# MerlinPCarson/WakeWord-Detection

Measured on AMD Instinct MI355X. Metric: audio frames/sec (16 kHz, 40-mel, 10 ms hop) + FRR@0.5 FA/h, higher is better.
Workload: dtype f32; 1 GPU; CRNN forward, batch=256x1.5 s synthetic 16 kHz clips per GPU, PCM resident in HBM -> log-mel (fp64 FFT) -> 151x40 window -> encode+detect, fp32 MFMA; clips_per_gpu=256, samples_per_clip=24000, resident_input_batches_rotated=24, resident_input_bytes=294912000, pipelined_contexts=4, weights=reference tf_lite_models (shipped fp32 weights), parallelism=single GPU

## Files before the change

wakeword-detection_amd/csrc/crnn.hip:

```cpp
#include "stream_fe.h"
#include <algorithm>
#include <type_traits>

#include <cstdlib>

typedef float f32x4 __attribute__((ext_vector_type(4)));

struct win_addr {
  const int64_t *row;
  const int32_t *valid;
  int64_t row0;
  int hop;
  int valid_const;
  int64_t mel_rows;
};

__device__ __forceinline__ void window_span(const win_addr &wa, int w, int T, int64_t &row, int &valid) {
  if (wa.row && wa.valid) {
    const int64_t r = wa.row[w];
    const int v = wa.valid[w];
    row = r;
    valid = v;
  } else {
    row = wa.row ? wa.row[w] : wa.row0 + (int64_t)w * wa.hop;
// ... 274 lines not shown
    load_a(av[0], 0);                                                                                \
    _Pragma("unroll") for (int i = 0; i < NT_; ++i) {                                                \
      if (i + 1 < NT_) load_a(av[(i + 1) & 1], i + 1);                                               \
      __builtin_amdgcn_sched_barrier(0);                                                             \
      f32x4 acc0 = {cb0, cb0, cb0, cb0}, acc1 = {cb1, cb1, cb1, cb1};                                \
      CV_MFMA_KB(av[i & 1], 0) CV_MFMA_KB(av[i & 1], 1) CV_MFMA_KB(av[i & 1], 2)                     \
      __builtin_amdgcn_sched_barrier(0);                                                             \
      __VA_ARGS__                                                                                    \
      __builtin_amdgcn_sched_barrier(0);                                                             \
      CV_MFMA_KB(av[i & 1], 3) CV_MFMA_KB(av[i & 1], 4) CV_MFMA_KB(av[i & 1], 5) CV_MFMA_LAST(av[i & 1]) \
      prev0 = acc0;                                                                                  \
      prev1 = acc1;                                                                                  \
    }                                                                                                \
  }

#define PJ_KS_BYTES (4 * 192 * 16)
typedef const __attribute__((address_space(1))) char *pj_gptr;
typedef const __attribute__((address_space(1))) f32x4 *pj_gptr4;
__device__ __forceinline__ float4 pj_w_ld(pj_gptr4 p) {
  const f32x4 v = *p;
  return make_float4(v.x, v.y, v.z, v.w);
}
#define PJ_W_LANE(wx1s_)                                                                             \
  const pj_gptr wb_0 = (pj_gptr)(wx1s_);                                                             \
  unsigned wb_lane = (unsigned)((kk * 192 + wave * 48 + j) * 16);
#define PJ_W_KSTEP(wk_, ks_)                                                                         \
  pj_gptr wk_ = wb_0 + (size_t)(ks_) * PJ_KS_BYTES;                                                  \
  asm("" : "+s"(wk_));                                                                               \
  asm("" : "+v"(wb_lane));
#define PJ_W_LD(wk_, n_) pj_w_ld((pj_gptr4)(wk_ + wb_lane + (n_) * 256))
#define PJ_RING_PROLOGUE(DEPTH_)                                                                     \
  _Pragma("unroll") for (int s2 = 0; s2 < DEPTH_ - 1; ++s2) {                                        \
    PJ_W_KSTEP(wk, s2)                                                                               \
    _Pragma("unroll") for (int n = 0; n < 3; ++n) bq[s2][n] = PJ_W_LD(wk, n);                        \
  }
#define PJ_LOAD_BIAS(bv1_, bx1_)                                                                     \
  _Pragma("unroll") for (int n = 0; n < 3; ++n) bv1_[n] = (bx1_)[wave * 48 + n * 16 + j];
#define PJ_ROWS16(e_)                                                                                \
  acc[0] = __builtin_amdgcn_mfma_f32_16x16x4f32(avq[ks & 1].e_, b[0].e_, acc[0], 0, 0, 0);            \
  acc[1] = __builtin_amdgcn_mfma_f32_16x16x4f32(avq[ks & 1].e_, b[1].e_, acc[1], 0, 0, 0);            \
  acc[2] = __builtin_amdgcn_mfma_f32_16x16x4f32(avq[ks & 1].e_, b[2].e_, acc[2], 0, 0, 0);
#define PJ_ROWS3(e_)                                                                                 \
  rem[0] = __builtin_amdgcn_mfma_f32_4x4x1f32(rvq[ks & 1].e_, b[0].e_, rem[0], 0, 0, 0);              \
  rem[1] = __builtin_amdgcn_mfma_f32_4x4x1f32(rvq[ks & 1].e_, b[1].e_, rem[1], 0, 0, 0);              \
  rem[2] = __builtin_amdgcn_mfma_f32_4x4x1f32(rvq[ks & 1].e_, b[2].e_, rem[2], 0, 0, 0);
#define PJ_NO_ROWS(e_)
#define PJ_KLOOP(DEPTH_, G16_, G3_, ...)                                                             \
  _Pragma("unroll") for (int ks = 0; ks < 40; ++ks) {                                                \
    if (ks + DEPTH_ - 1 < 40) {                                                                      \
      PJ_W_KSTEP(wk, ks + DEPTH_ - 1)                                                                \
      _Pragma("unroll") for (int n = 0; n < 3; ++n) bq[(ks + DEPTH_ - 1) % DEPTH_][n] = PJ_W_LD(wk, n); \
    }                                                                                                \
    if (ks + 1 < 40) { __VA_ARGS__ }                                                                 \
    __builtin_amdgcn_sched_barrier(0);                                                               \
    const float4 *b = bq[ks % DEPTH_];                                                               \
    G16_(x) G3_(x) G16_(y) G3_(y) G16_(z) G3_(z) G16_(w) G3_(w)                                      \
    __builtin_amdgcn_sched_barrier(0);                                                               \
  }
#define PJ_REM_ROWS(rem_, bv_, ...)                                                                  \
  _Pragma("unroll") for (int i = 0; i < 3; ++i) {                                                    \
    float s3 = rem_[i];                                                                              \
    s3 += __shfl_xor(s3, 16);                                                                        \
    s3 += __shfl_xor(s3, 32);                                                                        \
    if (kk == 0) {                                                                                   \
      const float v = s3 + bv_;                                                                      \
      __VA_ARGS__                                                                                    \
    }                                                                                                \
  }

#define CF_THREADS 256
#define CF_FLD 648
#define CF_IMG_FLOATS (CV_ROWS * CV_LDT)
#define CF_FEAT_FLOATS (CV_OT * CF_FLD)
#define CF_SMEM_BYTES ((CF_IMG_FLOATS + CF_FEAT_FLOATS) * 4)
#define CF_NO_ROW (-0x40000000)
#define CF_FUSED_FEAT_ROWS 13
#define CF_FUSED_SMEM_BYTES ((CF_IMG_FLOATS + CF_FUSED_FEAT_ROWS * CF_FLD) * 4)
#define CF_ALIAS_ROWS0 24
#define CF_ALIAS_REM (CF_ALIAS_ROWS0 + 3 * CF_FLD)
static_assert((((CF_ALIAS_ROWS0 - CF_IMG_FLOATS) / 4 - 2 * 13) % 16 + 16) % 16 == 0 && CF_IMG_FLOATS % 4 == 0, "aliased rows off their bank slots");
static_assert(CV_OT - 16 == 3 && 16 - CF_FUSED_FEAT_ROWS == 3 && CF_ALIAS_REM + 20 * 96 <= 20 * GR_GX_LD ,
              "the aliased rows must lie under gx");
#define CF_GX 0
#define CF_SEQ (20 * GR_GX_LD)
#define CF_HB (CF_SEQ + 32 * GR_SEQ_LD)
#define CF_ENC (CF_HB + 2 * 2 * 2 * GR_H)
#define CF_HID (CF_ENC + 2 * GR_H)
#define CF_W2S (CF_HID + 2 * GR_H)
static_assert(CF_W2S + 8 * 64 <= CF_IMG_FLOATS, "post-conv LDS layout exceeds the image region");
static_assert(64 * GR_W1_LD <= CF_FEAT_FLOATS && 16 * 192 * 4 <= CF_FEAT_FLOATS, "feat region too small for its later tenants");
static_assert(64 * GR_W1_LD <= CF_FUSED_FEAT_ROWS * CF_FLD, "fused kernel's feat region too small for the head's first layer");

struct fused_args {
  const float *mel;
  win_addr wa;
  const float *w4;
  const float *cbias;
  const float *wx1s;
  const float *bx1;
  const float *wh1, *bh1;
  const float *wx2s;
  const float *bx2, *wh2, *bh2, *w1, *b1, *w2, *b2;
  float *enc;
  float *out;
  int T, NOUT, HEAD;
  long long *stamps;
  float *gx_out;
  const unsigned short *cwb;
  const unsigned short *wx1b;
  ww_tick_tag tag;
};

template <bool SEQ>
__device__ __forceinline__ float cf_recurrence(const gru_w &g, const float *gxs, float *hd, float *seq1, int dir, int unit, int half) {
  constexpr int H = GR_H, OT = CV_OT;
  static_assert(OT % 2 == 1, "the step loop is pairs of steps plus one");
  const int t0 = dir ? OT - 1 : 0;
  const int gx_step = dir ? -GR_GX_LD : GR_GX_LD, seq_step = dir ? -GR_SEQ_LD : GR_SEQ_LD;
  const float *gxp = gxs + t0 * GR_GX_LD + dir * 3 * H + unit;
  float *sqp = SEQ ? seq1 + t0 * GR_SEQ_LD + dir * H + unit : nullptr;
  float *hw = hd + unit;
  float h_own = 0.f;
  float gz = gxp[0], gr = gxp[H], gc = gxp[2 * H];
#pragma unroll 1
  for (int s = 0; s < OT / 2; ++s) {
    float nz, nr, nc;
    gxp += gx_step;
    h_own = gru_step<true>(g, hd, half, gz, gr, gc, h_own, gxp, nz, nr, nc);
    if (half == 0) {
      hw[H] = h_own;
      if (SEQ) *sqp = h_own;
    }
    if (SEQ) sqp += seq_step;
    wsync_h();
    gxp += gx_step;
    h_own = gru_step<true>(g, hd + H, half, nz, nr, nc, h_own, gxp, gz, gr, gc);
    if (half == 0) {
      hw[0] = h_own;
      if (SEQ) *sqp = h_own;
    }
    if (SEQ) sqp += seq_step;
    wsync_h();
  }
  float nz, nr, nc;
  h_own = gru_step<false>(g, hd, half, gz, gr, gc, h_own, nullptr, nz, nr, nc);
  if (half == 0) {
    hw[H] = h_own;
    if (SEQ) *sqp = h_own;
  }
  wsync_h();
  return h_own;
}

#define CF_ROUND_L2(av_, rv_, b_, e_)                                                                  \
  acc[0] = __builtin_amdgcn_mfma_f32_16x16x4f32(av_.e_, b_[0].e_, acc[0], 0, 0, 0);                     \
  acc[1] = __builtin_amdgcn_mfma_f32_16x16x4f32(av_.e_, b_[1].e_, acc[1], 0, 0, 0);                     \
  acc[2] = __builtin_amdgcn_mfma_f32_16x16x4f32(av_.e_, b_[2].e_, acc[2], 0, 0, 0);                     \
  rem[0] = __builtin_amdgcn_mfma_f32_16x16x4f32(rv_.e_, b_[0].e_, rem[0], 0, 0, 0);                     \
  rem[1] = __builtin_amdgcn_mfma_f32_16x16x4f32(rv_.e_, b_[1].e_, rem[1], 0, 0, 0);                     \
  rem[2] = __builtin_amdgcn_mfma_f32_16x16x4f32(rv_.e_, b_[2].e_, rem[2], 0, 0, 0);

#define L2_LOAD_W(bq_, wx2s_, nt0_)                                                                  \
  _Pragma("unroll") for (int kb = 0; kb < 4; ++kb)                                                   \
    _Pragma("unroll") for (int n = 0; n < 3; ++n)                                                    \
      bq_[kb][n] = *(const float4 *)((wx2s_) + ((size_t)(kb * 4 + kk) * 192 + ((nt0_) + n) * 16 + j) * 4);
#define L2_LOAD_BIAS(bb_, bx2_, nt0_) \
  _Pragma("unroll") for (int n = 0; n < 3; ++n) bb_[n] = (bx2_)[((nt0_) + n) * 16 + j];
#define L2_PROJECT(bq_, bb_, rrow_, nt0_, ...)                                                       \
  {                                                                                                  \
    f32x4 acc[3] = {{0.f, 0.f, 0.f, 0.f}, {0.f, 0.f, 0.f, 0.f}, {0.f, 0.f, 0.f, 0.f}};               \
    f32x4 rem[3] = {{0.f, 0.f, 0.f, 0.f}, {0.f, 0.f, 0.f, 0.f}, {0.f, 0.f, 0.f, 0.f}};               \
    _Pragma("unroll") for (int kb = 0; kb < 4; ++kb) {                                               \
      const float4 av = *(const float4 *)(&seq1[j * GR_SEQ_LD + kb * 16 + kk * 4]);                  \
      const float4 rv = *(const float4 *)(&seq1[(rrow_) * GR_SEQ_LD + kb * 16 + kk * 4]);            \
      const float4 *b = bq_[kb];                                                                     \
      CF_ROUND_L2(av, rv, b, x) CF_ROUND_L2(av, rv, b, y) CF_ROUND_L2(av, rv, b, z) CF_ROUND_L2(av, rv, b, w) \
    }                                                                                                \
    __VA_ARGS__                                                                                      \
    _Pragma("unroll") for (int n = 0; n < 3; ++n) {                                                  \
      const int col = ((nt0_) + n) * 16 + j;                                                         \
      const float bb = bb_[n];                                                                       \
      _Pragma("unroll") for (int r = 0; r < 4; ++r) gxs[(kk * 4 + r) * GR_GX_LD + col] = acc[n][r] + bb; \
      if (kk == 0) {                                                                                 \
        _Pragma("unroll") for (int r = 0; r < 3; ++r) gxs[(16 + r) * GR_GX_LD + col] = rem[n][r] + bb; \
      }                                                                                              \
    }                                                                                                \
  }

__device__ __forceinline__ void cf_phases_d_to_g(const fused_args &a, float *img, float *feat, const gru_w &g, int w) {
  constexpr int H = GR_H;
  const int tid = threadIdx.x, lane = tid & 63, wave = wave_index(tid);
  const int j = lane & 15, kk = lane >> 4;
  const int unit = lane >> 1, half = lane & 1, dir = wave & 1;
  float *gxs = img + CF_GX, *seq1 = img + CF_SEQ, *hb = img + CF_HB, *encs = img + CF_ENC, *hid = img + CF_HID, *w2s = img + CF_W2S;
  float4 bq2[4][3];
  L2_LOAD_W(bq2, a.wx2s, wave * 3)
  if (wave < 2) {
    __builtin_amdgcn_s_setprio(3);
    cf_recurrence<true>(g, gxs, hb + dir * 2 * H, seq1, dir, unit, half);
    __builtin_amdgcn_s_setprio(0);
  }
  __syncthreads();

  {
    float bb2[3];
    L2_LOAD_BIAS(bb2, a.bx2, wave * 3)
    __builtin_amdgcn_sched_barrier(0);
    L2_PROJECT(bq2, bb2, 16 + j, wave * 3, )
  }
  __syncthreads();

  float *w1s = feat;
  if (wave >= 2) {
    __builtin_amdgcn_s_setprio(3);
    const float h_last = cf_recurrence<false>(g, gxs, hb + (2 + dir) * 2 * H, nullptr, dir, unit, half);
    __builtin_amdgcn_s_setprio(0);
    if (half == 0) {
      encs[dir * H + unit] = h_last;
      if (a.enc) a.enc[(size_t)w * 2 * H + dir * H + unit] = h_last;
    }
  } else {
    for (int i = tid; i < 64 * 64; i += 128) w1s[(i >> 6) * GR_W1_LD + (i & 63)] = a.w1[i];
    for (int i = tid; i < a.NOUT * 64; i += 128) w2s[i] = a.w2[i];
  }
  __syncthreads();

  if (wave == 0) {
    const float b1v = a.b1[lane], b2v = a.b2[lane < a.NOUT ? lane : 0];
    __builtin_amdgcn_sched_barrier(0);
    float acc = 0.f;
#pragma unroll 16
    for (int k = 0; k < 2 * H; ++k) acc = fmaf(w1s[lane * GR_W1_LD + k], encs[k], acc);
    hid[lane] = fmaxf(acc + b1v, 0.f);
    wsync_g();
    float y = 0.f;
    if (lane < a.NOUT) {
      for (int k = 0; k < 2 * H; ++k) y = fmaf(w2s[lane * 64 + k], hid[k], y);
      y += b2v;
    }
    const float p = head_activation(y, lane, a.NOUT, a.HEAD);
    if (a.tag.slots) {
      if (lane == a.tag.pidx) tick_tag_store(a.tag, w, p);
    } else if (lane < a.NOUT) {
      a.out[(size_t)w * a.NOUT + lane] = p;
    }
  }
}

#define CF_STAMP(i_) \
  if (FRONT_ONLY && a.stamps && lane == 0) a.stamps[((size_t)blockIdx.x * 4 + wave) * 10 + (i_)] = __builtin_amdgcn_s_memtime();
__device__ __forceinline__ void cf_set_move(fused_args &a, long long off) {
  ww_set_move(a.w4, off); ww_set_move(a.cbias, off); ww_set_move(a.wx1s, off); ww_set_move(a.bx1, off);
  ww_set_move(a.wh1, off); ww_set_move(a.bh1, off); ww_set_move(a.wx2s, off); ww_set_move(a.bx2, off);
  ww_set_move(a.wh2, off); ww_set_move(a.bh2, off); ww_set_move(a.w1, off); ww_set_move(a.b1, off);
  ww_set_move(a.w2, off); ww_set_move(a.b2, off); ww_set_move(a.cwb, off); ww_set_move(a.wx1b, off);
}
template <bool FRONT_ONLY, bool SET = false>
__global__ __launch_bounds__(CF_THREADS, 2) void crnn_fused_kernel(fused_args a, ww_set_ref set) {
  if constexpr (SET) cf_set_move(a, ww_set_offset(set, blockIdx.x));
  extern __shared__ __align__(16) float cf_smem[];
  float *img = cf_smem, *feat = cf_smem + CF_IMG_FLOATS;
  constexpr int H = GR_H, OT = CV_OT;
  const int tid = threadIdx.x, lane = tid & 63, wave = tid >> 6;
  const int j = lane & 15, kk = lane >> 4;
  const int w = blockIdx.x;
  CF_STAMP(0)
  int64_t row;
  int valid;
  window_span(a.wa, w, a.T, row, valid);

  float4 wreg[CV_KB][2];
  float wlast[2], cb0, cb1;
  CV_LOAD_W(wreg, wlast, cb0, cb1, a.w4, a.cbias)

  int a_off[6], o_off[6][4];
  {
    constexpr int MAXV = 6;
    const float *src = a.mel + row * CV_NMEL;
    const int n = valid * CV_NMEL;
    const bool al16 = ((((uintptr_t)src) & 15) == 0);
    float4 stage[MAXV];
    if (n > 0)
      stage_loads(al16, [&](auto al) {
        constexpr bool AL = decltype(al)::value;
#pragma unroll
        for (int q = 0; q < MAXV; ++q) {
          const int i = (q * CF_THREADS + tid) * 4;
          stage[q] = ld_mel4<AL>(src + (i < n ? i : n - 4), true);
        }
      });
    LDS_CLEAR16(img, CF_IMG_FLOATS / 4, CF_THREADS)
#pragma unroll
    for (int i = 0; i < 6; ++i) {
      constexpr int M = CV_OT * CV_OF;
      const int mt = wave + 4 * i;
      int m = mt * 16 + j;
      if (m >= M) m = M - 1;
      const int t = m / CV_OF, f = m - t * CV_OF;
      a_off[i] = (f * CV_SF) * CV_LDT + t * CV_ST;
#pragma unroll
      for (int r = 0; r < 4; ++r) {
        const int mo = mt * 16 + kk * 4 + r;
        const int to = mo / CV_OF, fo = mo - to * CV_OF;
        if (i < 4) o_off[i][r] = to * CF_FLD + fo * 32 + j;
        else if (i == 4) o_off[i][r] = (to < 13 ? to * CF_FLD : CF_ALIAS_ROWS0 - CF_IMG_FLOATS + (to - 13) * CF_FLD) + fo * 32 + j;
        else o_off[i][r] = mo >= M ? CF_NO_ROW : CF_ALIAS_REM - CF_IMG_FLOATS + fo * 96 + 16 * (to - 16) + j;
      }
    }
    __syncthreads();
#pragma unroll
    for (int q = 0; q < MAXV; ++q) {
      const int i = (q * CF_THREADS + tid) * 4;
      if (i < n) {
        const int it = i / CV_NMEL, im = i - it * CV_NMEL;
        float *d = img + (im + CV_PF) * CV_LDT + it + CV_PT;
        d[0] = stage[q].x;
        d[CV_LDT] = stage[q].y;
        d[2 * CV_LDT] = stage[q].z;
        d[3 * CV_LDT] = stage[q].w;
      }
    }
  }
  __syncthreads();
  CF_STAMP(1)
  PJ_W_LANE(a.wx1s)
  float4 bq[4][3];
  {
    auto load_a = [&](cv_a &av, int i) { CV_LOAD_A(av, img + a_off[i]) };
    auto store_tile = [&](int i, const f32x4 &r0, const f32x4 &r1) {
#pragma unroll
      for (int r = 0; r < 4; ++r) {
        if (i < 5) {
          feat[o_off[i][r]] = relu1(r0[r]);
          feat[o_off[i][r] + 16] = relu1(r1[r]);
        } else if (o_off[i][r] != CF_NO_ROW) {
          feat[o_off[i][r]] = relu1(r0[r]);
          feat[o_off[i][r] + 48] = relu1(r1[r]);
        }
      }
    };
    f32x4 prev0 = {0.f, 0.f, 0.f, 0.f}, prev1 = {0.f, 0.f, 0.f, 0.f}, t4_0 = prev0, t4_1 = prev0;
    CV_TILE_LOOP(6, if (i > 0 && i < 5) store_tile(i - 1, prev0, prev1); if (i == 5) { t4_0 = prev0; t4_1 = prev1; })
    PJ_RING_PROLOGUE(4)
    __builtin_amdgcn_sched_barrier(0);
    lds_barrier();
    store_tile(4, t4_0, t4_1);
    store_tile(5, prev0, prev1);
  }
  CF_STAMP(2)
  lds_barrier();
  CF_STAMP(3)
  float *gxs = img + CF_GX, *seq1 = img + CF_SEQ, *hb = img + CF_HB;
  CLEAR_SEQ_H(seq1, 32, hb, CF_THREADS)

  const int unit = lane >> 1, half = lane & 1, dir = wave & 1;
  gru_w g;
  {
    const float *a0p = (j < 13 ? feat + j * CF_FLD : img + CF_ALIAS_ROWS0 + (j - 13) * CF_FLD) + kk * 4;
    const int r1 = (lane & 3) < 3 ? (lane & 3) : 2;
    const float *a1p = img + CF_ALIAS_REM + 16 * r1 + kk * 4;
    f32x4 acc[3] = {{0.f, 0.f, 0.f, 0.f}, {0.f, 0.f, 0.f, 0.f}, {0.f, 0.f, 0.f, 0.f}};
// ... 502 lines not shown
          const bf16x8_t wh = __builtin_bit_cast(bf16x8_t, wq[0][ks][mt]), wl = __builtin_bit_cast(bf16x8_t, wq[1][ks][mt]);
          acc[mt] = __builtin_amdgcn_mfma_f32_16x16x32_bf16(wl, xh[i & 1][ks], acc[mt], 0, 0, 0);
          acc[mt] = __builtin_amdgcn_mfma_f32_16x16x32_bf16(wh, xl[i & 1][ks], acc[mt], 0, 0, 0);
          acc[mt] = __builtin_amdgcn_mfma_f32_16x16x32_bf16(wh, xh[i & 1][ks], acc[mt], 0, 0, 0);
        }
      if (i > 0) store_pos(i - 1, prev);
      prev[0] = acc[0];
      prev[1] = acc[1];
    }
    store_pos(5, prev);
  }
  auto w_ld = [&](int p, int ks, int n) { return ((const uint4 *)a.wx1b)[((size_t)(p * WX1B_KS + ks) * WX1B_NT + wave * 3 + n) * 64 + lane]; };
  uint4 bq[3][2][3];
#pragma unroll
  for (int s2 = 0; s2 < 2; ++s2)
#pragma unroll
    for (int p = 0; p < 2; ++p)
#pragma unroll
      for (int n = 0; n < 3; ++n) bq[s2][p][n] = w_ld(p, s2, n);
  __syncthreads();
  float *gxs = img + CF_GX, *seq1 = img + CF_SEQ, *hb = img + CF_HB;
  for (int i = tid; i < 32 * GR_SEQ_LD; i += CF_THREADS) seq1[i] = 0.f;
  if (tid < 2 * 2 * 2 * H) hb[tid] = 0.f;

  const int unit = lane >> 1, half = lane & 1, dir = wave & 1;
  gru_w g;
  {
    const int r1 = 16 + j < OT ? 16 + j : OT - 1;
    const unsigned short *a0h = fth + j * CB_FLD + kk * 8, *a0l = ftl + j * CB_FLD + kk * 8;
    const unsigned short *a1h = fth + r1 * CB_FLD + kk * 8, *a1l = ftl + r1 * CB_FLD + kk * 8;
    f32x4 acc[2][3];
#pragma unroll
    for (int mt = 0; mt < 2; ++mt)
#pragma unroll
      for (int n = 0; n < 3; ++n) acc[mt][n] = (f32x4){0.f, 0.f, 0.f, 0.f};
    float bv1[3];
#pragma unroll
    for (int n = 0; n < 3; ++n) bv1[n] = a.bx1[wave * 48 + n * 16 + j];
    if (!FRONT_ONLY) gru_load_w(g, wave < 2 ? a.wh1 : a.wh2, wave < 2 ? a.bh1 : a.bh2, dir, unit, half);
#pragma unroll
    for (int ks = 0; ks < 20; ++ks) {
      if (ks + 2 < 20) {
#pragma unroll
        for (int p = 0; p < 2; ++p)
#pragma unroll
          for (int n = 0; n < 3; ++n) bq[(ks + 2) % 3][p][n] = w_ld(p, ks + 2, n);
      }
      const bf16x8_t ah[2] = {*(const bf16x8_t *)(a0h + ks * 32), *(const bf16x8_t *)(a1h + ks * 32)};
      const bf16x8_t al[2] = {*(const bf16x8_t *)(a0l + ks * 32), *(const bf16x8_t *)(a1l + ks * 32)};
#pragma unroll
      for (int n = 0; n < 3; ++n) {
        const bf16x8_t bh = __builtin_bit_cast(bf16x8_t, bq[ks % 3][0][n]), bl = __builtin_bit_cast(bf16x8_t, bq[ks % 3][1][n]);
#pragma unroll
        for (int mt = 0; mt < 2; ++mt) {
          acc[mt][n] = __builtin_amdgcn_mfma_f32_16x16x32_bf16(al[mt], bh, acc[mt][n], 0, 0, 0);
          acc[mt][n] = __builtin_amdgcn_mfma_f32_16x16x32_bf16(ah[mt], bl, acc[mt][n], 0, 0, 0);
          acc[mt][n] = __builtin_amdgcn_mfma_f32_16x16x32_bf16(ah[mt], bh, acc[mt][n], 0, 0, 0);
        }
      }
    }
#pragma unroll
    for (int n = 0; n < 3; ++n) {
      const int col = wave * 48 + n * 16 + j;
      const float bv = bv1[n];
#pragma unroll
      for (int mt = 0; mt < 2; ++mt)
#pragma unroll
        for (int r = 0; r < 4; ++r) {
          const int t = mt * 16 + kk * 4 + r;
          if (t < OT) gxs[t * GR_GX_LD + col] = acc[mt][n][r] + bv;
        }
    }
  }
  __syncthreads();
  if (FRONT_ONLY) {
    float4 *dst = (float4 *)(a.gx_out + (size_t)w * OT * 6 * H);
    for (int q = tid; q < OT * 6 * H / 4; q += CF_THREADS) {
      const int e = q * 4, t = e / (6 * H), c = e - t * 6 * H;
      dst[q] = *(const float4 *)(&gxs[t * GR_GX_LD + c]);
    }
    return;
  }
  cf_phases_d_to_g(a, img, feat, g, w);
}

struct tail_args {
  const float *gx1;
  const float *wh1, *bh1;
  const float *wx2s;
  const float *bx2, *wh2, *bh2, *w1, *b1, *w2, *b2;
  float *enc, *out;
  int NOUT, HEAD;
  const float *gxI, *gxL, *gxR;
  int hop_g, eight_g;
  const int64_t *iI0;
  const float *wx2;
};
#define GT_SEQ (19 * GR_GX_LD)
#define GT_HB (GT_SEQ + 20 * GR_SEQ_LD)
#define GT_ENC (GT_HB + 2 * 2 * 2 * GR_H)
#define GT_HID (GT_ENC + 2 * GR_H)
#define GT_SMEM_FLOATS (GT_HID + 2 * GR_H)

__device__ __forceinline__ void gt_set_move(tail_args &a, const ww_set_ref &set, int slot) {
  const long long off = ww_set_offset(set, slot);
  ww_set_move(a.wh1, off); ww_set_move(a.bh1, off); ww_set_move(a.wx2s, off); ww_set_move(a.wx2, off); ww_set_move(a.bx2, off);
  ww_set_move(a.wh2, off); ww_set_move(a.bh2, off); ww_set_move(a.w1, off); ww_set_move(a.b1, off); ww_set_move(a.w2, off);
  ww_set_move(a.b2, off);
  const size_t nI = (size_t)set.aux[WW_SLIDE_AUX_NI], nW = (size_t)set.aux[WW_SLIDE_AUX_NW], W = (size_t)set.aux[WW_SLIDE_AUX_W];
  a.gxI += (size_t)slot * nI * 6 * GR_H;
  a.gxL += (size_t)slot * nW * 6 * GR_H;
  a.gxR += (size_t)slot * nW * 6 * GR_H;
  a.out += (size_t)slot * W * a.NOUT;
}

template <bool SET = false>
__global__ __launch_bounds__(128, 4) void gru_tail_kernel(tail_args a, ww_set_ref set) {
  if constexpr (SET) gt_set_move(a, set, blockIdx.y);
  constexpr int H = GR_H, OT = CV_OT;
  __shared__ __align__(16) float sm[GT_SMEM_FLOATS];
  float *gxs = sm, *seq1 = sm + GT_SEQ, *hb = sm + GT_HB, *encs = sm + GT_ENC, *hid = sm + GT_HID;
  const int tid = threadIdx.x, lane = tid & 63, dir = wave_index(tid);
  const int j = lane & 15, kk = lane >> 4, unit = lane >> 1, half = lane & 1;
  const int w = blockIdx.x;
  gru_w g;
  gru_load_w(g, a.wh1, a.bh1, dir, unit, half);
  {
    constexpr int NQ = OT * 6 * H / 4, NS = (NQ + 127) / 128;
    int64_t i0w = (int64_t)w * a.hop_g;
    if (!a.gx1 && a.iI0) i0w = a.iI0[w];
    f32x4 st[NS];
#pragma unroll
    for (int s = 0; s < NS; ++s) {
      const int q = min(tid + 128 * s, NQ - 1), t = q / 48, c4 = q - t * 48;
      const float *row = a.gx1 ? a.gx1 + ((size_t)w * OT + t) * 6 * H
                       : t == 0 ? a.gxL + (size_t)w * 6 * H
                       : t == OT - 1 ? a.gxR + (size_t)w * 6 * H
                                     : a.gxI + ((size_t)i0w + (size_t)(t - 1) * a.eight_g) * 6 * H;
      st[s] = *(const f32x4 *)(row + c4 * 4);
    }
#pragma unroll
    for (int s = 0; s < NS; ++s) {
      const int q = tid + 128 * s, t = q / 48, c4 = q - t * 48;
      if (q < NQ) *(f32x4 *)(&gxs[t * GR_GX_LD + c4 * 4]) = st[s];
    }
  }
  CLEAR_SEQ_H(seq1, 20, hb, 128)
  __syncthreads();
  cf_recurrence<true>(g, gxs, hb + dir * 2 * H, seq1, dir, unit, half);
  __syncthreads();
#pragma unroll 1
  for (int pass = 0; pass < 2; ++pass) {
    const int nt0 = dir * 6 + pass * 3;
    float4 bq[4][3];
    L2_LOAD_W(bq, a.wx2s, nt0)
    float bb2[3];
    L2_LOAD_BIAS(bb2, a.bx2, nt0)
    L2_PROJECT(bq, bb2, j < 3 ? 16 + j : 19 , nt0, __syncthreads();)
  }
  gru_w g2;
  gru_load_w(g2, a.wh2, a.bh2, dir, unit, half);
  __syncthreads();
  const float h_last = cf_recurrence<false>(g2, gxs, hb + (2 + dir) * 2 * H, nullptr, dir, unit, half);
  if (half == 0) {
    encs[dir * H + unit] = h_last;
    if (a.enc) a.enc[(size_t)w * 2 * H + dir * H + unit] = h_last;
  }
  __syncthreads();
  if (dir == 0) {
    const float b1v = a.b1[lane], b2v = a.b2[lane < a.NOUT ? lane : 0];
    float acc = 0.f;
    const float4 *wr = (const float4 *)(a.w1 + (size_t)lane * 2 * H);
#pragma unroll
    for (int q = 0; q < 16; ++q) {
      const float4 wv = wr[q];
      const float4 ev = *(const float4 *)(&encs[q * 4]);
      acc = fmaf(wv.x, ev.x, acc); acc = fmaf(wv.y, ev.y, acc);
      acc = fmaf(wv.z, ev.z, acc); acc = fmaf(wv.w, ev.w, acc);
    }
    hid[lane] = fmaxf(acc + b1v, 0.f);
    wsync_g();
    float y = 0.f;
    if (lane < a.NOUT) {
      for (int k = 0; k < 2 * H; ++k) y = fmaf(a.w2[lane * 64 + k], hid[k], y);
      y += b2v;
    }
    const float p = head_activation(y, lane, a.NOUT, a.HEAD);
    if (lane < a.NOUT) a.out[(size_t)w * a.NOUT + lane] = p;
  }
}

#define GT16_LD 36
#define GT16_ELD 68
#define GT16_SMEM_BYTES ((2 * 2 * 16 * GT16_LD + 2 * 6 * 2 * 64 * 4) * 4)
struct tail16_args {
  tail_args t;
  float *seq;
  int nw;
};

template <bool SET = false>
__global__ __launch_bounds__(128, 2) void gru_tail16_kernel(tail16_args aa, ww_set_ref set) {
  if constexpr (SET) {
    gt_set_move(aa.t, set, blockIdx.y);
    aa.seq += (size_t)blockIdx.y * (size_t)((aa.nw + 15) / 16) * CV_OT * 16 * 2 * GR_H;
  }
  constexpr int H = GR_H, OT = CV_OT;
  const tail_args &a = aa.t;
  extern __shared__ __align__(16) float sm16[];
  float (*hs)[2][16 * GT16_LD] = (float (*)[2][16 * GT16_LD])sm16;
  float *encs = sm16 + 2 * 2 * 16 * GT16_LD, *hid = encs + 16 * GT16_ELD;
  static_assert(2 * 16 * GT16_ELD <= 2 * 6 * 2 * 64 * 4, "enc / hid rows do not fit the weight pages");
  const int tid = threadIdx.x, lane = tid & 63, dir = tid >> 6;
  const int c = lane & 15, g = lane >> 4;
  float4 *whl = (float4 *)(sm16 + 2 * 2 * 16 * GT16_LD) + (size_t)dir * 6 * 2 * 64 + lane;
  const int w0 = blockIdx.x * 16;
  float *seq = aa.seq + (size_t)blockIdx.x * OT * 16 * 2 * H;

  int wi[4];
  int64_t i0[4];
#pragma unroll
  for (int r = 0; r < 4; ++r) wi[r] = min(w0 + 4 * g + r, aa.nw - 1);
  if (!a.gx1 && a.iI0) {
#pragma unroll
    for (int r = 0; r < 4; ++r) i0[r] = a.iI0[wi[r]];
  } else {
#pragma unroll
    for (int r = 0; r < 4; ++r) i0[r] = a.gx1 ? 0 : (int64_t)wi[r] * a.hop_g;
  }
  auto gx_row = [&](int r, int t) -> const float * {
    if (a.gx1) return a.gx1 + ((size_t)wi[r] * OT + t) * 6 * H;
    if (t == 0) return a.gxL + (size_t)wi[r] * 6 * H;
    if (t == OT - 1) return a.gxR + (size_t)wi[r] * 6 * H;
    return a.gxI + (size_t)(i0[r] + (int64_t)(t - 1) * a.eight_g) * 6 * H;
  };
#define GT16_POS(u_) (8 * (((u_) >> 1) & 3) + 4 * ((u_) >> 4) + 2 * (((u_) >> 3) & 1) + ((u_) & 1))
  float bh[6];
  auto load_wh = [&](const float *whp, const float *bhp) {
#pragma unroll
    for (int nt = 0; nt < 6; ++nt) {
      const int row = (nt >> 1) * H + (nt & 1) * 16 + c;
      const float *p = whp + ((size_t)dir * 3 * H + row) * H + 2 * g;
      float wv[8];
#pragma unroll
      for (int i = 0; i < 8; ++i) wv[i] = p[16 * (i >> 2) + 8 * ((i >> 1) & 1) + (i & 1)];
      whl[(2 * nt) * 64] = make_float4(wv[0], wv[1], wv[2], wv[3]);
      whl[(2 * nt + 1) * 64] = make_float4(wv[4], wv[5], wv[6], wv[7]);
      bh[nt] = bhp[dir * 3 * H + row];
    }
  };
#define GT16_PRE_ALL(X0_)                                                                          \
  {                                                                                                \
    float4 wb[2][2];                                                                               \
    wb[0][0] = whl[0];                                                                             \
    wb[0][1] = whl[64];                                                                            \
    _Pragma("unroll") for (int nt = 0; nt < 6; ++nt) {                                             \
      if (nt + 1 < 6) {                                                                            \
        wb[(nt + 1) & 1][0] = whl[(2 * nt + 2) * 64];                                              \
        wb[(nt + 1) & 1][1] = whl[(2 * nt + 3) * 64];                                              \
      }                                                                                            \
      __builtin_amdgcn_sched_barrier(0);                                                           \
      const float4 b0 = wb[nt & 1][0], b1 = wb[nt & 1][1];                                         \
      f32x4 e0 = nt < 4 ? X0_[nt < 4 ? nt : 0] : zero4, o0 = {bh[nt], bh[nt], bh[nt], bh[nt]};     \
      e0 = __builtin_amdgcn_mfma_f32_16x16x4f32(ha[0], b0.x, e0, 0, 0, 0);                         \
      o0 = __builtin_amdgcn_mfma_f32_16x16x4f32(ha[1], b0.y, o0, 0, 0, 0);                         \
      e0 = __builtin_amdgcn_mfma_f32_16x16x4f32(ha[2], b0.z, e0, 0, 0, 0);                         \
      o0 = __builtin_amdgcn_mfma_f32_16x16x4f32(ha[3], b0.w, o0, 0, 0, 0);                         \
      f32x4 e1 = zero4, o1 = zero4;                                                                \
      e1 = __builtin_amdgcn_mfma_f32_16x16x4f32(ha[4], b1.x, e1, 0, 0, 0);                         \
      o1 = __builtin_amdgcn_mfma_f32_16x16x4f32(ha[5], b1.y, o1, 0, 0, 0);                         \
      e1 = __builtin_amdgcn_mfma_f32_16x16x4f32(ha[6], b1.z, e1, 0, 0, 0);                         \
      o1 = __builtin_amdgcn_mfma_f32_16x16x4f32(ha[7], b1.w, o1, 0, 0, 0);                         \
      pre[nt] = (e0 + o0) + (e1 + o1);                                                             \
      __builtin_amdgcn_sched_barrier(0);                                                           \
    }                                                                                              \
  }
#define GT16_PRE_FIRST(X0_)                                                                        \
  _Pragma("unroll") for (int nt = 0; nt < 6; ++nt) {                                               \
    const f32x4 o0 = {bh[nt], bh[nt], bh[nt], bh[nt]};                                             \
    pre[nt] = ((nt < 4 ? X0_[nt < 4 ? nt : 0] : zero4) + o0) + (zero4 + zero4);                    \
  }
  load_wh(a.wh1, a.bh1);
  for (int i = tid; i < 2 * 2 * 16 * GT16_LD; i += 128) (&hs[0][0][0])[i] = 0.f;
  const int pos0 = GT16_POS(c), pos1 = GT16_POS(16 + c);

  float h_own[4][2];
#pragma unroll
  for (int r = 0; r < 4; ++r) h_own[r][0] = h_own[r][1] = 0.f;
  float gxn[4][6];
  {
    const int t = dir ? OT - 1 : 0;
#pragma unroll
    for (int r = 0; r < 4; ++r) {
      const float *row = gx_row(r, t) + dir * 3 * H + c;
#pragma unroll
      for (int nt = 0; nt < 6; ++nt) gxn[r][nt] = row[(nt >> 1) * H + (nt & 1) * 16];
    }
  }
  __syncthreads();
#pragma unroll 1
  for (int s = 0; s < OT; ++s) {
    const int t = dir ? OT - 1 - s : s, cur = s & 1;
    f32x4 x0[4];
#pragma unroll
    for (int nt = 0; nt < 4; ++nt) x0[nt] = (f32x4){gxn[0][nt], gxn[1][nt], gxn[2][nt], gxn[3][nt]};
    float gxc[4][2];
#pragma unroll
    for (int r = 0; r < 4; ++r) { gxc[r][0] = gxn[r][4]; gxc[r][1] = gxn[r][5]; }
    if (s + 1 < OT) {
      const int tn = dir ? t - 1 : t + 1;
#pragma unroll
      for (int r = 0; r < 4; ++r) {
        const float *row = gx_row(r, tn) + dir * 3 * H + c;
#pragma unroll
// ... 572 lines not shown
```

Measured before the change: 926.5 million audio frames/s.

## Compute remainder rows of layer-2 projection with 4x4x1 MFMA blocks

The three leftover time rows (rows 16-18) of the layer-2 GRU input projection were computed with full 16x16x4 MFMAs, which wasted most of their lanes. They are now computed with 4x4x1f32 MFMAs in broadcast mode, interleaved with the main 16x16 MFMAs over a skewed five-step loop. The remainder weights are double-buffered and loaded one step ahead, and sched_barriers pin the issue order. This cuts the number of MFMA issues for the remainder, but it adds more weight loads and registers and makes the schedule more complex.

```diff
diff --git a/wakeword-detection_amd/csrc/crnn.hip b/wakeword-detection_amd/csrc/crnn.hip
--- a/wakeword-detection_amd/csrc/crnn.hip
+++ b/wakeword-detection_amd/csrc/crnn.hip
@@ -450,38 +450,53 @@
   return h_own;
 }
 
-#define CF_ROUND_L2(av_, rv_, b_, e_)                                                                  \
-  acc[0] = __builtin_amdgcn_mfma_f32_16x16x4f32(av_.e_, b_[0].e_, acc[0], 0, 0, 0);                     \
-  acc[1] = __builtin_amdgcn_mfma_f32_16x16x4f32(av_.e_, b_[1].e_, acc[1], 0, 0, 0);                     \
-  acc[2] = __builtin_amdgcn_mfma_f32_16x16x4f32(av_.e_, b_[2].e_, acc[2], 0, 0, 0);                     \
-  rem[0] = __builtin_amdgcn_mfma_f32_16x16x4f32(rv_.e_, b_[0].e_, rem[0], 0, 0, 0);                     \
-  rem[1] = __builtin_amdgcn_mfma_f32_16x16x4f32(rv_.e_, b_[1].e_, rem[1], 0, 0, 0);                     \
-  rem[2] = __builtin_amdgcn_mfma_f32_16x16x4f32(rv_.e_, b_[2].e_, rem[2], 0, 0, 0);
+#define CF_ROUND_L2(e_, i_)                                                                          \
+  if (s < 4) acc[0] = __builtin_amdgcn_mfma_f32_16x16x4f32(av.e_, b[0].e_, acc[0], 0, 0, 0);          \
+  if (s > 0) rem = __builtin_amdgcn_mfma_f32_4x4x1f32(ra, rb[0].e_, rem, 4, 0 + i_, 0);               \
+  __builtin_amdgcn_sched_barrier(0);                                                                 \
+  if (s < 4) acc[1] = __builtin_amdgcn_mfma_f32_16x16x4f32(av.e_, b[1].e_, acc[1], 0, 0, 0);          \
+  if (s > 0) rem = __builtin_amdgcn_mfma_f32_4x4x1f32(ra, rb[1].e_, rem, 4, 4 + i_, 0);               \
+  __builtin_amdgcn_sched_barrier(0);                                                                 \
+  if (s < 4) acc[2] = __builtin_amdgcn_mfma_f32_16x16x4f32(av.e_, b[2].e_, acc[2], 0, 0, 0);          \
+  if (s > 0) rem = __builtin_amdgcn_mfma_f32_4x4x1f32(ra, rb[2].e_, rem, 4, 8 + i_, 0);               \
+  __builtin_amdgcn_sched_barrier(0);                                                                 \
+  if (s > 0) rem = __builtin_amdgcn_mfma_f32_4x4x1f32(ra, rb[3].e_, rem, 4, 12 + i_, 0);              \
+  __builtin_amdgcn_sched_barrier(0);
 
 #define L2_LOAD_W(bq_, wx2s_, nt0_)                                                                  \
   _Pragma("unroll") for (int kb = 0; kb < 4; ++kb)                                                   \
     _Pragma("unroll") for (int n = 0; n < 3; ++n)                                                    \
       bq_[kb][n] = *(const float4 *)((wx2s_) + ((size_t)(kb * 4 + kk) * 192 + ((nt0_) + n) * 16 + j) * 4);
-#define L2_LOAD_BIAS(bb_, bx2_, nt0_) \
-  _Pragma("unroll") for (int n = 0; n < 3; ++n) bb_[n] = (bx2_)[((nt0_) + n) * 16 + j];
-#define L2_PROJECT(bq_, bb_, rrow_, nt0_, ...)                                                       \
+#define L2_REM_COL(nt0_) ((nt0_) * 16 + (lane < 48 ? lane : 47))
+#define L2_LOAD_WR(rq_, wx2s_, nt0_, kb_)                                                            \
+  _Pragma("unroll") for (int q = 0; q < 4; ++q)                                                      \
+    rq_[q] = *(const float4 *)((wx2s_) + ((size_t)((kb_) * 4 + q) * 192 + L2_REM_COL(nt0_)) * 4);
+#define L2_LOAD_BIAS(bb_, bx2_, nt0_)                                                                \
+  _Pragma("unroll") for (int n = 0; n < 3; ++n) bb_[n] = (bx2_)[((nt0_) + n) * 16 + j];              \
+  bb_[3] = (bx2_)[L2_REM_COL(nt0_)];
+#define L2_PROJECT(bq_, rq_, bb_, wx2s_, nt0_, ...)                                                  \
   {                                                                                                  \
     f32x4 acc[3] = {{0.f, 0.f, 0.f, 0.f}, {0.f, 0.f, 0.f, 0.f}, {0.f, 0.f, 0.f, 0.f}};               \
-    f32x4 rem[3] = {{0.f, 0.f, 0.f, 0.f}, {0.f, 0.f, 0.f, 0.f}, {0.f, 0.f, 0.f, 0.f}};               \
-    _Pragma("unroll") for (int kb = 0; kb < 4; ++kb) {                                               \
-      const float4 av = *(const float4 *)(&seq1[j * GR_SEQ_LD + kb * 16 + kk * 4]);                  \
-      const float4 rv = *(const float4 *)(&seq1[(rrow_) * GR_SEQ_LD + kb * 16 + kk * 4]);            \
-      const float4 *b = bq_[kb];                                                                     \
-      CF_ROUND_L2(av, rv, b, x) CF_ROUND_L2(av, rv, b, y) CF_ROUND_L2(av, rv, b, z) CF_ROUND_L2(av, rv, b, w) \
+    f32x4 rem = {0.f, 0.f, 0.f, 0.f};                                                                \
+    const float *rrow = &seq1[(16 + (lane & 3)) * GR_SEQ_LD + (lane >> 2)];                          \
+    _Pragma("unroll") for (int s = 0; s < 5; ++s) {                                                  \
+      float4 av;                                                                                     \
+      float ra;                                                                                      \
+      if (s < 4) av = *(const float4 *)(&seq1[j * GR_SEQ_LD + s * 16 + kk * 4]);                     \
+      if (s > 0) ra = rrow[(s - 1) * 16];                                                            \
+      const float4 *b = bq_[s & 3], *rb = rq_[(s + 1) & 1];                                          \
+      CF_ROUND_L2(x, 0) CF_ROUND_L2(y, 1) CF_ROUND_L2(z, 2) CF_ROUND_L2(w, 3)                        \
+      if (s < 3) { L2_LOAD_WR(rq_[(s + 1) & 1], wx2s_, nt0_, s + 1) }                                \
+      __builtin_amdgcn_sched_barrier(0);                                                             \
     }                                                                                                \
     __VA_ARGS__                                                                                      \
     _Pragma("unroll") for (int n = 0; n < 3; ++n) {                                                  \
       const int col = ((nt0_) + n) * 16 + j;                                                         \
       const float bb = bb_[n];                                                                       \
       _Pragma("unroll") for (int r = 0; r < 4; ++r) gxs[(kk * 4 + r) * GR_GX_LD + col] = acc[n][r] + bb; \
-      if (kk == 0) {                                                                                 \
-        _Pragma("unroll") for (int r = 0; r < 3; ++r) gxs[(16 + r) * GR_GX_LD + col] = rem[n][r] + bb; \
-      }                                                                                              \
+    }                                                                                                \
+    if (lane < 48) {                                                                                 \
+      _Pragma("unroll") for (int r = 0; r < 3; ++r) gxs[(16 + r) * GR_GX_LD + (nt0_) * 16 + lane] = rem[r] + bb_[3]; \
     }                                                                                                \
   }
 
@@ -501,10 +516,12 @@
   __syncthreads();
 
   {
-    float bb2[3];
+    float bb2[4];
+    float4 rq2[2][4];
+    L2_LOAD_WR(rq2[0], a.wx2s, wave * 3, 0)
     L2_LOAD_BIAS(bb2, a.bx2, wave * 3)
     __builtin_amdgcn_sched_barrier(0);
-    L2_PROJECT(bq2, bb2, 16 + j, wave * 3, )
+    L2_PROJECT(bq2, rq2, bb2, a.wx2s, wave * 3, )
   }
   __syncthreads();
 
@@ -1313,14 +1330,17 @@
 #pragma unroll 1
   for (int pass = 0; pass < 2; ++pass) {
     const int nt0 = dir * 6 + pass * 3;
-    float4 bq[4][3];
+    float4 bq[4][3], rq[2][4];
     L2_LOAD_W(bq, a.wx2s, nt0)
-    float bb2[3];
+    L2_LOAD_WR(rq[0], a.wx2s, nt0, 0)
+    float bb2[4];
     L2_LOAD_BIAS(bb2, a.bx2, nt0)
-    L2_PROJECT(bq, bb2, j < 3 ? 16 + j : 19 , nt0, __syncthreads();)
+    L2_PROJECT(bq, rq, bb2, a.wx2s, nt0, __syncthreads();)
   }
   gru_w g2;
-  gru_load_w(g2, a.wh2, a.bh2, dir, unit, half);
+  int lane2 = lane;
+  asm("" : "+v"(lane2));
+  gru_load_w(g2, a.wh2, a.bh2, dir, lane2 >> 1, lane2 & 1);
   __syncthreads();
   const float h_last = cf_recurrence<false>(g2, gxs, hb + (2 + dir) * 2 * H, nullptr, dir, unit, half);
   if (half == 0) {
```

Result: no change. 931.7 million audio frames/s, median of 6 (+0.6%).
